# leonsick/depthg

Hardware: AMD Instinct MI355X
Metric: correlation-loss steps/sec at B=32,C=384,28x28 (fwd+bwd, per-GPU batch 32) (higher is better)
Workload: dtype bf16 (feats) / f16 (code) MFMA inputs, f32 accumulate

## Files before the change

depthg_amd/csrc/dg_api_corr.hip:

```cpp
#include "dg_api.h"
#include "dg_corr_args.h"
#include "dg_taps.h"

static unsigned long long* g_prof_span = nullptr;
extern "C" int dg_prof_main_span(void* span) { g_prof_span = static_cast<unsigned long long*>(span); return DG_OK; }

enum class Prep { Small, Dense, General };
enum class Sampler { Plane, ChannelLast };
enum class MainKernel { Small, Corr2, CorrMain };
enum class Depth { None, Job, GsBlocks, GsOwnLaunch };
enum class Hist { Rows, Blobs };
enum class Masks { None, Sampled, DenseRaw, DenseSplit };

struct PairSet {
    int op;
    int neg;
    bool mapped;
    float shift;
    int slot_loss, slot_cd;
    float fin_scale;
    int gidx, csel, dest;
    float factor;
};
struct Operand {
// ... 19 lines not shown
    float shift_depth;
    float inv_numel;
    float grad_f, grad_fn;
    int blob, blob_off_c;
    PairSet ps[DG_MAX_NEG + 2];
    Operand ops[DG_MAX_NEG + 2];
    bool gr_on;
    int gr_nkeys, gr_cpb, gr_blocks_per_image;
    int8_t gr_key[DG_MAX_JOBS], gr_first[DG_MAX_JOBS];
    int32_t gr_nblk[DG_MAX_JOBS];
    size_t nhwc_f[2], nhwc_c[2];
    size_t rows_f[DG_MAX_NEG + 2], rows_c[DG_MAX_NEG + 2];
    size_t op[DG_MAX_NEG + 2], inv[DG_MAX_NEG + 2], colpart[DG_MAX_NEG + 2], bbar[DG_MAX_NEG + 2];
    size_t ccolpart[DG_MAX_NEG + 2], csum[DG_MAX_NEG + 2], bsplit[DG_MAX_NEG + 2];
    size_t rvec[DG_MAX_NEG + 2], rimg[DG_MAX_NEG + 2];
    size_t nz, nzsum;
    size_t dRA[DG_MAX_NEG + 3], dRB[DG_MAX_NEG + 2];
    size_t part[DG_MAX_NEG + 3];
    size_t comb[2], scratch_out, taps, gbuf[DG_MAX_NEG + 2];
    size_t ticket;
    size_t maskbits[DG_MAX_NEG + 2];
    size_t clo[2];
    size_t gr_list, gr_count, gr_rank;
    size_t dRA2[DG_MAX_NEG + 2], dRBs[DG_MAX_NEG + 2], dRB2[DG_MAX_NEG + 2][2], dRBm[DG_MAX_NEG + 2], part4, om;
    size_t total;

    bool small() const { return prep == Prep::Small; }
    bool dense() const { return prep == Prep::Dense; }
    bool plane() const { return sampler == Sampler::Plane; }
    bool has_masks() const { return masks != Masks::None; }
    bool depth_in_gs() const { return depth_run == Depth::GsBlocks || depth_run == Depth::GsOwnLaunch; }
    bool dense_masks() const { return masks == Masks::DenseRaw || masks == Masks::DenseSplit; }
    bool intra_symmetric() const { return !pointwise || fold; }
    const int64_t* batch_map(int k, const int64_t* perms) const {
        return k < 0 ? nullptr : reinterpret_cast<const int64_t*>(reinterpret_cast<uintptr_t>(perms) + (size_t)k * B * sizeof(int64_t));
    }
    const int64_t* map_of(int t, const int64_t* perms) const { return batch_map(ps[t].mapped ? ps[t].neg : -1, perms); }
};

static inline float* f32(char* ws, size_t off) { return reinterpret_cast<float*>(ws + off); }

#define FOLD_STASH_OFF (5 * 1024)

static void plan_tables(const dg_corr_desc* d, Plan& p) {
    const double numel = (double)p.B * p.P * p.P;
    p.inv_numel = (float)(1.0 / numel);
// ... 109 lines not shown
    for (int i = 0; i < 2; ++i) p.comb[i] = take(B * p.Ppad * p.KD * 4);
    p.scratch_out = take(DG_OUT_COUNT * 4);
    p.taps = take(2 * B * dg_taps_record_bytes(p.hc * p.wc, p.P));
    for (int t = 0; t < p.T; ++t) p.gbuf[t] = p.grad ? take(B * (size_t)(p.Ppad / 32) * (p.Ppad / 32) * 2048) : 0;
    p.ticket = take(256);
    const bool xmask = rows && !p.small() && p.grad && plain_zero_clamp && p.Ppad <= 256 && p.rf == 4;
    const bool xmask_dense = (d->flags & DG_EXACT_MASKS) && ident && p.grad && plain_zero_clamp &&
                             p.KF == 384 && p.KD == 96 && p.D <= 80 && p.Ppad >= 160 && p.B <= 64;
    if ((d->flags & DG_EXACT_MASKS) && p.grad && (d->flags & DG_ZERO_CLAMP) && !xmask && !xmask_dense && !p.small())
        return fail(DG_ERR_UNSUPPORTED, "DG_EXACT_MASKS: exact clamp masks exist on small sample grids (always on there) and on the dense "
                                        "identity grid with C <= 384 (padded to 384), D <= 80, P >= 160, B <= 64, zero_clamp without stabalize");
    p.masks = xmask ? Masks::Sampled : (!xmask_dense ? Masks::None : (p.pointwise ? Masks::DenseSplit : Masks::DenseRaw));
    for (int t = 0; t < p.T; ++t) p.maskbits[t] = take(p.has_masks() ? B * (size_t)(p.Ppad / 32) * p.Ppad * 4 : 0);
    p.main = p.small() ? MainKernel::Small
                       : (p.grad && dg_corr2_shape_supported(p.KF, p.KD, p.D, p.lo, p.hi, p.Ppad, p.B) ? MainKernel::Corr2 : MainKernel::CorrMain);
    static const bool fold_on = [] { const char* e = getenv("DG_FOLD_INTRA"); return !(e && e[0] == '0'); }();
    p.fold = fold_on && p.main == MainKernel::Corr2 && p.pointwise && !xmask;
    p.half = p.main == MainKernel::Corr2 && ident && p.N * p.B <= 512 && p.S == p.h && p.S == p.w;
    p.depth_run = (!p.depth || p.small()) ? Depth::None : (!p.grad ? Depth::Job : (p.dense_masks() ? Depth::GsOwnLaunch : Depth::GsBlocks));
    for (int i = 0; i < 2; ++i) p.clo[i] = take(p.masks == Masks::DenseSplit ? B * (size_t)(p.Ppad / 32) * p.KD * 64 : 0);
    p.gr_list = take((size_t)DG_MAX_JOBS * B * DG_GR_CAP * 4);
    p.gr_count = take((size_t)DG_MAX_JOBS * B * 4);
    p.gr_rank = take((size_t)DG_MAX_JOBS * B * 2);
    {
        const bool sg = p.small() && p.grad, two = sg && p.pointwise;
        const size_t gt = B * p.Ppad * p.KD * 4;
        for (int t = 0; t < p.T; ++t) {
            p.dRA2[t] = take(two ? gt : 0);
            p.dRBs[t] = take(sg && p.nsplit == 2 ? gt : 0);
            for (int k = 0; k < 2; ++k) p.dRB2[t][k] = take(two && k < p.nsplit ? gt : 0);
            p.dRBm[t] = take(sg && t >= 2 && (p.pointwise || p.nsplit == 2) ? gt : 0);
        }
        p.part4 = take(p.small() ? (size_t)(p.T + 1) * B * p.nsplit * 16 : 0);
        p.om = take(p.small() ? (size_t)(p.T + 1) * 4 : 0);
    }
    p.total = off;
    plan_tables(d, p);
    return DG_OK;
}

extern "C" size_t dg_corr_workspace_bytes(const dg_corr_desc* desc) {
    Plan p{};
    if (make_plan(desc, p) != DG_OK) return 0;
    return p.total;
}

// ... 310 lines not shown
    DG_HIP(dg_launch_gather(g, p.KF, c.stream));
    return DG_OK;
}

static int fwd_colmeans(Fwd& c) {
    const Plan& p = c.p;
    const DgCorrArgs& a = c.a;
    DgColmeanArgs m;
    memset(&m, 0, sizeof(m));
    m.nops = p.nops; m.B = p.B; m.P = p.P; m.Ppad = p.Ppad; m.KF = p.KF; m.KD = p.KD;
    for (int o = 0; o < p.nops; ++o) {
        m.colpart[o] = p.pointwise ? f32(c.ws, p.colpart[o]) : nullptr; m.bbar[o] = f32(c.ws, p.bbar[o]);
        m.bsplit[o] = reinterpret_cast<__bf16*>(c.ws + p.bsplit[o]);
        m.ngroups[o] = p.Ppad / 32;
        m.ccolpart[o] = f32(c.ws, p.ccolpart[o]); m.csum[o] = f32(c.ws, p.csum[o]);
    }
    m.zero_word = p.depth_in_gs() ? reinterpret_cast<unsigned int*>(c.ws + p.ticket) : nullptr;
    m.zero_words9 = a.wctr;
    if (p.gr_on) {
        m.gr.nh = p.T; m.gr.nkeys = p.gr_nkeys; m.gr.B = p.B;
        for (int t = 0; t < p.T; ++t) { m.gr.sidx[t] = p.map_of(t, c.perms); m.gr.key[t] = p.gr_key[t]; }
        m.gr.list = reinterpret_cast<int32_t*>(c.ws + p.gr_list); m.gr.count = reinterpret_cast<int32_t*>(c.ws + p.gr_count);
        m.gr.rank = reinterpret_cast<int16_t*>(c.ws + p.gr_rank);
    }
    if (p.dense() && p.pointwise) {
        m.dc.code[0] = c.code; m.dc.code[1] = c.code_pos;
        for (int o = 0; o < 2; ++o) { m.dc.blob[o] = c.ws + p.op[o]; m.dc.inv_norm[o] = f32(c.ws, p.inv[o]); m.dc.ccolpart[o] = f32(c.ws, p.ccolpart[o]); }
        m.dc.B = p.B; m.dc.D = p.D; m.dc.KF = p.KF; m.dc.KD = p.KD; m.dc.h = p.h; m.dc.w = p.w; m.dc.P = p.P; m.dc.Ppad = p.Ppad;
        if (p.masks == Masks::DenseSplit) { m.dc.clo[0] = c.ws + p.clo[0]; m.dc.clo[1] = c.ws + p.clo[1]; }
    }
    if (c.split) {
        DgColmeanArgs ms = m;
        ms.zsel = 1; m.zsel = 2;
        DG_HIP(c.side->hand_over(0));
        DG_HIP(dg_launch_colmean(ms, c.side->stream()));
    }
    DG_HIP(dg_launch_colmean(m, c.stream));
    return DG_OK;
}

static int fwd_cd_mask3(Fwd& c) {
    const Plan& p = c.p;
    DgCdMask3Args m;
    memset(&m, 0, sizeof(m));
    m.opR = c.ws + p.op[0]; m.loR = c.ws + p.clo[0];
    for (int t = 0; t < p.T; ++t) {
// ... 220 lines not shown
    if (!p.grad) return fail(DG_ERR_INVALID, "dg_corr_backward needs a descriptor with DG_NEED_GRAD (as used in forward)");
    if (!coords1 || !coords2 || !grad_code || !grad_code_pos || !workspace) return fail(DG_ERR_INVALID, "null pointer");
    if (p.N > 0 && !perms) return fail(DG_ERR_INVALID, "perms is null with n_neg=%d", p.N);
    if (workspace_bytes < p.total) return fail(DG_ERR_WORKSPACE, "workspace %zu < required %zu bytes", workspace_bytes, p.total);
    char* ws = static_cast<char*>(workspace);
    DgScatterArgs s;
    memset(&s, 0, sizeof(s));
    ScatterFill fill{s, ws};
    if (p.small()) scatter_sources_small(p, perms, fill);
    else scatter_sources_blobs(p, perms, fill);
    if (p.depth) fill.add(p.dRA[p.T], nullptr, 3, 0, 2.0f * p.grad_f, 0, 1);
    s.coords1 = coords1; s.coords2 = coords2; s.gscal = grad_scalars; s.gtot = grad_total;
    s.wtot[0] = desc->w_intra; s.wtot[1] = desc->w_inter; s.wtot[2] = desc->w_neg; s.wtot[3] = desc->w_depth;
    s.comb[0] = f32(ws, p.comb[0]); s.comb[1] = f32(ws, p.comb[1]);
    s.taps = ws + p.taps;
    s.xop = ws + p.op[0]; s.xinv = f32(ws, p.inv[0]); s.blob_bytes = p.blob; s.blob_off_c = p.blob_off_c;
    s.xinv_dest[0] = f32(ws, p.inv[0]); s.xinv_dest[1] = p.nops > 1 ? f32(ws, p.inv[1]) : nullptr;
    s.out[0] = grad_code; s.out[1] = grad_code_pos;
    s.B = p.B; s.D = p.D; s.DP = p.KD; s.h = p.hc; s.w = p.wc; s.S = p.S; s.Sh = p.Sh; s.P = p.P; s.Ppad = p.Ppad;
    if ((size_t)p.hc * p.wc > 4096) return fail(DG_ERR_UNSUPPORTED, "code map %dx%d too large for the gradient gather (max 4096 pixels)", p.hc, p.wc);
    s.DC = 8;
    s.dense = p.dense() ? 1 : 0;
    s.taps_ready = p.dense() ? 0 : 1;
    DG_HIP(dg_launch_scatter(s, static_cast<hipStream_t>(stream_)));
    return DG_OK;
}

extern "C" int dg_corr_backward(const dg_corr_desc* desc, const float* grad_scalars, const float* coords1,
                                const float* coords2, const int64_t* perms, float* grad_code, float* grad_code_pos,
                                void* workspace, size_t workspace_bytes, dg_stream_t stream_) {
    if (!grad_scalars) return fail(DG_ERR_INVALID, "null pointer");
    return corr_backward_impl(desc, grad_scalars, nullptr, coords1, coords2, perms, grad_code, grad_code_pos, workspace,
                              workspace_bytes, stream_);
}

extern "C" int dg_corr_backward_total(const dg_corr_desc* desc, const float* grad_total, const float* coords1,
                                      const float* coords2, const int64_t* perms, float* grad_code, float* grad_code_pos,
                                      void* workspace, size_t workspace_bytes, dg_stream_t stream_) {
    if (!grad_total) return fail(DG_ERR_INVALID, "null pointer");
    return corr_backward_impl(desc, nullptr, grad_total, coords1, coords2, perms, grad_code, grad_code_pos, workspace,
                              workspace_bytes, stream_);
}

static int materialize_impl(const dg_corr_desc* desc, int32_t which, const int64_t* perms, float* out_cd, float* out_loss,
                            void* workspace, size_t workspace_bytes, dg_stream_t stream_) {
    Plan p{};
// ... 80 lines not shown
    int rc = make_plan(desc, p);
    if (rc != DG_OK) return rc;
    if (!workspace || workspace_bytes < p.total) return fail(DG_ERR_WORKSPACE, "workspace missing or too small");
    if (p.N > 0 && !perms) return fail(DG_ERR_INVALID, "perms is null");
    char* ws = static_cast<char*>(workspace);
    if (p.small()) {
        DgSmallArgs m;
        small_args(p, desc, ws, perms, m);
        m.out = f32(ws, p.scratch_out);
        DG_HIP(dg_launch_corr_small(m, static_cast<hipStream_t>(stream_)));
        return DG_OK;
    }
    DgCorrArgs a;
    build_corr_jobs(p, ws, perms, a);
    return launch_main(p, a, static_cast<hipStream_t>(stream_));
}

extern "C" int dg_corr_intra_folded(const dg_corr_desc* desc) {
    Plan p{};
    if (make_plan(desc, p) != DG_OK) return -1;
    return p.fold ? 1 : 0;
}

extern "C" const char* dg_corr_main_kernel_name(const dg_corr_desc* desc) {
    Plan p{};
    if (make_plan(desc, p) != DG_OK) return nullptr;
    return p.main == MainKernel::Small ? "k_corr_small" : (p.main == MainKernel::Corr2 ? "k_corr2" : "k_corr_main");
}

extern "C" int dg_normalize_split(int32_t B, int32_t C, int32_t h, int32_t w, const float* src, int32_t nchunks, int32_t chunk_c,
                                  float* const* dst, dg_stream_t stream_) {
    if (B < 1 || C < 1 || h < 1 || w < 1 || !src || !dst) return fail(DG_ERR_INVALID, "dg_normalize_split: bad arguments");
    if (nchunks < 1 || nchunks > 16 || chunk_c < 1 || (long long)chunk_c * (nchunks - 1) >= C || (long long)chunk_c * nchunks < C)
        return fail(DG_ERR_INVALID, "dg_normalize_split: %d chunks of %d channels do not tile C=%d (at most 16 chunks)", nchunks, chunk_c, C);
    for (int k = 0; k < nchunks; ++k) if (!dst[k]) return fail(DG_ERR_INVALID, "dg_normalize_split: null destination %d", k);
    DG_HIP(dg_launch_normalize_split(src, B, C, h * w, nchunks, chunk_c, dst, static_cast<hipStream_t>(stream_)));
    return DG_OK;
}
```

depthg_amd/csrc/dg_corr_args.h:

```cpp
#pragma once
#include "dg_device.h"

__host__ __device__ inline int dg_perm32(int pl) {
    int s = pl >> 4, u = (pl >> 3) & 1, hh = (pl >> 2) & 1, v = pl & 3;
    return (2 * s + hh) * 8 + 4 * u + v;
}

#ifndef DG_F_IG
#define DG_F_IG 4
#endif
__host__ __device__ inline int dg_f_off(int q, int g) {
    constexpr int IG = DG_F_IG;
    return ((g / IG) * 32 + q) * (IG * 16) + (((g % IG) ^ ((q / (16 / IG)) % IG)) * 16);
}

struct DgBlob {
    int GF, GD, KD;
    int off_c, off_p, bytes;
    __host__ __device__ DgBlob(int KF, int KD_) : GF(KF / 8), GD(KD_ / 8), KD(KD_) {
        off_c = 32 * GF * 16;
        off_p = off_c + GD * 32 * 16;
        bytes = off_p + 4 * KD * 16;
    }
    __host__ __device__ int f(int q, int g) const { return dg_f_off(q, g); }
// ... 315 lines not shown
    const int B = g.B;
    int src[DG_MAX_JOBS];
#pragma unroll
    for (int j = 0; j < DG_MAX_JOBS; ++j) {
        const bool mine = j < g.nh && g.key[j] == key && lane < B;
        const int64_t* sidx = mine ? g.sidx[j] : nullptr;
        src[j] = mine ? (sidx ? (int)sidx[lane] : lane) : -1;
    }
    int cnt = 0;
#pragma unroll
    for (int j = 0; j < DG_MAX_JOBS; ++j) {
        const bool hit = src[j] == m;
        const unsigned long long mask = __ballot(hit);
        if (hit) {
            const int rk = cnt + __popcll(mask & ((1ull << lane) - 1ull));
            g.rank[j * B + lane] = (int16_t)(rk < 32767 ? rk : 32767);
            if (rk < DG_GR_CAP) g.list[(key * B + m) * DG_GR_CAP + rk] = j | (lane << 8);
        }
        cnt += __popcll(mask);
    }
    if (lane == 0) g.count[key * B + m] = cnt < DG_GR_CAP ? cnt : DG_GR_CAP;
}

struct DgColmeanArgs {
    const float* colpart[DG_MAX_NEG + 2];
    float* bbar[DG_MAX_NEG + 2];
    __bf16* bsplit[DG_MAX_NEG + 2];
    const float* ccolpart[DG_MAX_NEG + 2];
    float* csum[DG_MAX_NEG + 2];
    int32_t ngroups[DG_MAX_NEG + 2];
    int32_t nops, B, P, Ppad, KF, KD;
    unsigned int* zero_word;
    unsigned int* zero_words9;
    DgGroupArgs gr;
    DgDenseCodeArgs dc;
    int32_t zsel;
};

struct DgRowmeanJob {
    const char* A;
    const float* bbar;
    const __bf16* bsplit;
    const int64_t* aidx;
    const int64_t* bidx;
    float* rvec;
    float* rimg;
};
struct DgRowmeanArgs {
    DgRowmeanJob jobs[DG_MAX_NEG + 2];
    int32_t njobs, B, P, Ppad, KF, KD;
    const float* abar;
    char* stash;
    int32_t stash_off;
    const float* cs_part[2];
    float* cs_out[2];
    int32_t ncs;
};
// ... 12 lines not shown
#define DG_MAX_SCATTER 48
struct DgScatterArgs {
    DgScatterSrc src[DG_MAX_SCATTER];
    int32_t nsrc;
    const float* coords1;
    const float* coords2;
    const float* gscal;
    const float* gtot;
    float wtot[4];
    float* comb[2];
    char* taps;
    const char* xop;
    const float* xinv;
    const float* xinv_dest[2];
    int32_t blob_bytes, blob_off_c;
    float* out[2];
    int32_t B, D, DP, h, w, S, Sh, P, Ppad, DC;
    int32_t dense;
    int8_t craw[2][DG_MAX_SCATTER / 2], cfin[2][DG_MAX_SCATTER / 2];
    int8_t ncraw[2], ncfin[2];
    int8_t crawh[2][DG_MAX_SCATTER / 2], cfinh[2][DG_MAX_SCATTER / 2];
    int8_t ncrawh[2], ncfinh[2];
    int32_t routed_half;
    int32_t taps_ready;
    int32_t naxpy;
    float* axo[DG_MAX_NEG + 2];
    const float* axd[DG_MAX_NEG + 2];
    const float* axd2[DG_MAX_NEG + 2];
    const float* axs[DG_MAX_NEG + 2];
    const float* axs2[DG_MAX_NEG + 2];
    const float* axf[DG_MAX_NEG + 2];
};

__device__ __forceinline__ float dg_src_factor(const DgScatterSrc& q) { return q.dfac ? q.factor * q.dfac[0] : q.factor; }
__device__ __forceinline__ float dg_gscal(const DgScatterArgs& a, int i) {
    return a.gscal ? a.gscal[i] + a.gscal[DG_OUT_TOTAL] * a.wtot[i] : a.gtot[0] * a.wtot[i];
}

struct DgGsJob {
    const uint16_t* G;
    const char* Rop;
    const char* Sop;
    const float* ScInv;
    const int64_t* ridx;
    const int64_t* sidx;
    float* dS;
// ... 66 lines not shown
```

depthg_amd/csrc/dg_post.hip:

```cpp
#include "dg_device.h"
#include "dg_corr_args.h"
#include "dg_taps.h"
#include <cstdlib>

typedef const float __attribute__((address_space(1)))* gfloat_p;


#define DG_LOAD_GS(a, gs)                                                                                   \
    float gs[4];                                                                                            \
    {                                                                                                       \
        const bool vec_ = (a).gscal != nullptr;                                                             \
        const float gt_ = vec_ ? (a).gscal[DG_OUT_TOTAL] : (a).gtot[0];                                     \
        const float g0_ = vec_ ? (a).gscal[0] : 0.f, g1_ = vec_ ? (a).gscal[1] : 0.f;                       \
        const float g2_ = vec_ ? (a).gscal[2] : 0.f, g3_ = vec_ ? (a).gscal[3] : 0.f;                       \
        gs[0] = g0_ + gt_ * (a).wtot[0]; gs[1] = g1_ + gt_ * (a).wtot[1];                                  \
        gs[2] = g2_ + gt_ * (a).wtot[2]; gs[3] = g3_ + gt_ * (a).wtot[3];                                  \
    }
__device__ __forceinline__ float dg_pick(const float (&gs)[4], int i) { return i == 0 ? gs[0] : (i == 1 ? gs[1] : (i == 2 ? gs[2] : gs[3])); }

template <int NDF>
__global__ __launch_bounds__(64 * NDF) void k_grad_combine(const DgScatterArgs a) {
    const int rt = blockIdx.x, n = blockIdx.y, dest = blockIdx.z;
    const int lane = threadIdx.x & 63, r = lane & 31, h = lane >> 5, DP = NDF * 32;
    const int d = __builtin_amdgcn_readfirstlane((int)threadIdx.x >> 6);
// ... 73 lines not shown
            v[i] = (v[i] - (float)x[0][i] * t) * inv;
        }
    }
    add_sources(a.cfin[dest], a.ncfin[dest]);
    if (ok) {
        float* out = a.comb[dest] + tile_off;
#pragma unroll
        for (int g = 0; g < 4; ++g) {
            const f32x4 t = {v[4 * g], v[4 * g + 1], v[4 * g + 2], v[4 * g + 3]};
            *reinterpret_cast<f32x4*>(out + g * 256) = t;
        }
    }
}

#ifndef COMB_HB_HM
#define COMB_HB_HM 4
#endif
#ifndef COMB_HB
#define COMB_HB 4
#endif
#define COMB_MAXROUTE 512
template <int NDF, bool HM = false>
__global__ __launch_bounds__(64 * NDF) void k_combine_out(const DgScatterArgs a) {
    const int rt = blockIdx.x, n = blockIdx.y, dest = blockIdx.z;
    const int tid = threadIdx.x, lane = tid & 63, r = lane & 31, h = lane >> 5, DP = NDF * 32;
    const int d = __builtin_amdgcn_readfirstlane(tid >> 6);
    __shared__ __attribute__((aligned(16))) char xs[NDF][DG_XROWS_LDS];
    __shared__ float part[NDF][32];
    __shared__ float stage[NDF][32 * 33];
    __shared__ const float* rl_p[COMB_MAXROUTE];
    __shared__ float rl_w[COMB_MAXROUTE];
    __shared__ int rl_cnt, wcnt[NDF], rsrc[DG_MAX_SCATTER];
    DG_LOAD_GS(a, gs)
    int nr = 0;
    for (int s = 0; s < a.nsrc; ++s)
        if (a.src[s].dest == dest && a.src[s].route != nullptr) { if (tid == 0) rsrc[nr] = s; ++nr; }
    if (tid == 0) rl_cnt = 0;
    __syncthreads();
    for (int i0 = 0; i0 < nr * a.B; i0 += 64 * NDF) {
        const int i = i0 + tid;
        bool hit = false;
        int m = 0, s = 0;
        if (i < nr * a.B) {
            const int rs = i / a.B;
            m = i - rs * a.B; s = rsrc[rs];
            hit = (int)a.src[s].route[m] == n;
        }
        const unsigned long long bal = __ballot(hit);
        if (lane == 0) wcnt[d] = __popcll(bal);
        __syncthreads();
        int base = rl_cnt;
        for (int wv = 0; wv < d; ++wv) base += wcnt[wv];
        if (hit) {
            const int o = base + __popcll(bal & ((1ull << lane) - 1));
            const DgScatterSrc& q = a.src[s];
            if (o < COMB_MAXROUTE) {
                rl_p[o] = q.half ? reinterpret_cast<const float*>(reinterpret_cast<const _Float16*>(q.buf) + (size_t)m * a.Ppad * a.DP) : q.buf + (size_t)m * a.Ppad * a.DP;
                rl_w[o] = dg_src_factor(q) * dg_pick(gs, q.gidx);
            }
        }
        __syncthreads();
        if (tid == 0) {
            int c = rl_cnt;
            for (int wv = 0; wv < NDF; ++wv) c += wcnt[wv];
            rl_cnt = min(c, COMB_MAXROUTE);
        }
        __syncthreads();
    }
    const int cnt = rl_cnt;
    const bool ok = 32 * d + r < a.D;
    const size_t in_img = (size_t)rt * (32 * DP) + lane * 4 + (ok ? d * 1024 : 0);
    const size_t tile_off = (size_t)n * a.Ppad * DP + in_img;
    float v[16];
#pragma unroll
    for (int i = 0; i < 16; ++i) v[i] = 0.f;
    const size_t in_img_h = (size_t)rt * (32 * DP) + lane * 8 + (ok ? d * 1024 : 0);
    constexpr int HB = HM ? COMB_HB_HM : COMB_HB, FB = HM ? 1 : 4;
    float invd[16];
#pragma unroll
    for (int i = 0; i < 16; ++i) {
        const int rr = rt * 32 + (i & 3) + 8 * (i >> 2) + 4 * h;
        invd[i] = (a.xinv_dest[dest] && rr < a.P) ? a.xinv_dest[dest][(size_t)n * a.Ppad + rr] : 0.f;
    }
    const _Float16 __attribute__((address_space(1)))* const hdummy = reinterpret_cast<const _Float16 __attribute__((address_space(1)))*>(reinterpret_cast<uintptr_t>(a.xinv));
    auto add_half4 = [&](const _Float16 __attribute__((address_space(1)))* const (&hb)[HB], const float (&sc)[HB], const bool raw) __attribute__((always_inline)) {
        f16x8 t0[HB], t1[HB];
#pragma unroll
        for (int u = 0; u < HB; ++u) {
            t0[u] = *reinterpret_cast<const f16x8 __attribute__((address_space(1)))*>(hb[u]);
            t1[u] = *reinterpret_cast<const f16x8 __attribute__((address_space(1)))*>(hb[u] + ((ok && hb[u] != hdummy) ? 512 : 0));
        }
#pragma unroll
        for (int u = 0; u < HB; ++u) {
            const bool use = ok && sc[u] != 0.f;
#pragma unroll
            for (int e = 0; e < 8; ++e) {
                v[e] = fmaf(raw ? sc[u] : sc[u] * invd[e], use ? (float)t0[u][e] : 0.f, v[e]);
                v[8 + e] = fmaf(raw ? sc[u] : sc[u] * invd[8 + e], use ? (float)t1[u][e] : 0.f, v[8 + e]);
            }
        }
    };
    auto add_sources_half = [&](const int8_t* list, const int nsrc_, const bool raw) __attribute__((always_inline)) {
        for (int k0 = 0; k0 < nsrc_; k0 += HB) {
            const _Float16 __attribute__((address_space(1)))* hb[HB];
            float sc[HB];
#pragma unroll
            for (int u = 0; u < HB; ++u) {
                const bool live = k0 + u < nsrc_;
                const DgScatterSrc& q = a.src[(int)list[live ? k0 + u : k0]];
                sc[u] = live ? dg_src_factor(q) * dg_pick(gs, q.gidx) : 0.f;
                hb[u] = live ? reinterpret_cast<const _Float16 __attribute__((address_space(1)))*>(reinterpret_cast<uintptr_t>(q.buf)) + (size_t)n * a.Ppad * DP + in_img_h
                             : hdummy;
            }
            add_half4(hb, sc, raw);
        }
    };
    auto add_sources = [&](const int8_t* list, const int nsrc_) __attribute__((always_inline)) {

        for (int k0 = 0; k0 < nsrc_; k0 += FB) {
            f32x4 t[FB][4];
            float sc[FB];
#pragma unroll
            for (int u = 0; u < FB; ++u) {
                const bool live = k0 + u < nsrc_;
                const DgScatterSrc& q = a.src[(int)list[live ? k0 + u : k0]];
                sc[u] = live ? dg_src_factor(q) * dg_pick(gs, q.gidx) : 0.f;
                const float* base = q.buf + tile_off;
#pragma unroll
                for (int g = 0; g < 4; ++g) t[u][g] = *reinterpret_cast<const f32x4*>(base + (ok ? g * 256 : 0));
            }
#pragma unroll
            for (int u = 0; u < FB; ++u) {
                const bool use = ok && k0 + u < nsrc_;
#pragma unroll
                for (int g = 0; g < 4; ++g)
#pragma unroll
                    for (int e = 0; e < 4; ++e) v[4 * g + e] = fmaf(sc[u], use ? t[u][g][e] : 0.f, v[4 * g + e]);
            }
        }
    };
    const int nraw = a.ncraw[dest] + a.ncrawh[dest];
    add_sources(a.craw[dest], a.ncraw[dest]);
    add_sources_half(a.crawh[dest], a.ncrawh[dest], true);
    if (nraw > 0) {
        const char* xb = a.xop + ((size_t)n * (a.Ppad >> 5) + rt) * a.blob_bytes + a.blob_off_c + d * 2048;
        _Float16 x[1][16];
        dg_load_code_rows<1>(xb, xs[d], lane, x);
#pragma unroll
        for (int i = 0; i < 16; ++i) {
            const float t = half_sum((float)x[0][i] * v[i]);
            if (r == 0) part[d][h * 16 + i] = t;
        }
        __syncthreads();
#pragma unroll
        for (int i = 0; i < 16; ++i) {
            float t = part[0][h * 16 + i];
#pragma unroll
            for (int f = 1; f < NDF; ++f) t += part[f][h * 16 + i];
            const int rr = rt * 32 + (i & 3) + 8 * (i >> 2) + 4 * h;
            const float inv = rr < a.P ? a.xinv[(size_t)n * a.Ppad + rr] : 0.f;
            v[i] = (v[i] - (float)x[0][i] * t) * inv;
        }
    }
    add_sources(a.cfin[dest], a.ncfin[dest]);
    add_sources_half(a.cfinh[dest], a.ncfinh[dest], false);
    if (a.routed_half) {
        for (int e0 = 0; e0 < cnt; e0 += HB) {
            const _Float16 __attribute__((address_space(1)))* hb[HB];
            float sc[HB];
#pragma unroll
            for (int k = 0; k < HB; ++k) {
                const int e = min(e0 + k, cnt - 1);
                sc[k] = e0 + k < cnt ? rl_w[e] : 0.f;
                hb[k] = sc[k] != 0.f ? reinterpret_cast<const _Float16 __attribute__((address_space(1)))*>(reinterpret_cast<uintptr_t>(rl_p[e])) + in_img_h : hdummy;
            }
            add_half4(hb, sc, false);
        }
    } else
    for (int e0 = 0; e0 < cnt; e0 += 4) {
        f32x4 u4[4][4];
        float sc[4];
#pragma unroll
        for (int k = 0; k < 4; ++k) {
            const int e = min(e0 + k, cnt - 1);
            sc[k] = e0 + k < cnt ? rl_w[e] : 0.f;
            const gfloat_p sb = (gfloat_p)rl_p[e] + in_img;
#pragma unroll
            for (int g = 0; g < 4; ++g) u4[k][g] = *(const f32x4 __attribute__((address_space(1)))*)(sb + (ok ? g * 256 : 0));
        }
#pragma unroll
        for (int k = 0; k < 4; ++k)
#pragma unroll
            for (int g = 0; g < 4; ++g)
#pragma unroll
                for (int e = 0; e < 4; ++e) v[4 * g + e] = fmaf(sc[k], ok ? u4[k][g][e] : 0.f, v[4 * g + e]);
    }
    float* st = stage[d];
#pragma unroll
    for (int i = 0; i < 16; ++i) st[r * 33 + (i & 3) + 8 * (i >> 2) + 4 * h] = v[i];
    __builtin_amdgcn_fence(__ATOMIC_RELEASE, "workgroup");
    __builtin_amdgcn_wave_barrier();
    __builtin_amdgcn_fence(__ATOMIC_ACQUIRE, "workgroup");
    const int HW = a.h * a.w, p = rt * 32 + r;
    float* out = a.out[dest] + (size_t)n * a.D * HW + p;
#pragma unroll
    for (int it = 0; it < 16; ++it) {
        const int c = 2 * it + h, ch = 32 * d + c;
        if (ch < a.D && p < a.P) out[(size_t)ch * HW] = st[c * 33 + r];
    }
// ... 364 lines not shown

hipError_t dg_launch_scatter(const DgScatterArgs& a, hipStream_t s) {
    DgScatterArgs ac = a;
    {
        for (int dest = 0; dest < 2; ++dest) {
            ac.ncraw[dest] = ac.ncfin[dest] = ac.ncrawh[dest] = ac.ncfinh[dest] = 0;
            for (int i = 0; i < a.nsrc; ++i) {
                const DgScatterSrc& q = a.src[i];
                if (q.dest != dest || q.route != nullptr) continue;
                int8_t& cnt = q.half ? (q.raw ? ac.ncrawh[dest] : ac.ncfinh[dest]) : (q.raw ? ac.ncraw[dest] : ac.ncfin[dest]);
                if (cnt >= DG_MAX_SCATTER / 2) return hipErrorInvalidValue;
                (q.half ? (q.raw ? ac.crawh[dest] : ac.cfinh[dest]) : (q.raw ? ac.craw[dest] : ac.cfin[dest]))[cnt++] = (int8_t)i;
            }
        }
        const dim3 cgrid(a.Ppad / 32, a.B, 2);
        {
            int nrouted = 0;
            for (int i = 0; i < a.nsrc; ++i) nrouted += a.src[i].route != nullptr;
            bool any_half = false;
            int routed_h = 0;
            for (int i = 0; i < a.nsrc; ++i) { any_half = any_half || a.src[i].half != 0; routed_h += (a.src[i].route != nullptr && a.src[i].half) ? 1 : 0; }
            if (routed_h != 0 && routed_h != nrouted) return hipErrorInvalidValue;
            ac.routed_half = routed_h != 0 ? 1 : 0;
            const bool one_launch = a.dense && a.S == a.h && a.S == a.w && nrouted * a.B <= COMB_MAXROUTE && (a.DP == 96 || a.DP == 128);
            if (any_half && !one_launch) return hipErrorInvalidValue;
            if (one_launch) {
                if (a.DP == 96 && any_half) hipLaunchKernelGGL((k_combine_out<3, true>), cgrid, dim3(192), 0, s, ac);
                else if (a.DP == 96) hipLaunchKernelGGL(k_combine_out<3>, cgrid, dim3(192), 0, s, ac);
                else hipLaunchKernelGGL(k_combine_out<4>, cgrid, dim3(256), 0, s, ac);
                return hipGetLastError();
            }
        }
        const dim3 cgrid2(a.Ppad / 32, a.B, 2 + a.naxpy);
        if (a.DP == 96) hipLaunchKernelGGL(k_grad_combine<3>, cgrid2, dim3(192), 0, s, ac);
        else if (a.DP == 128) hipLaunchKernelGGL(k_grad_combine<4>, cgrid2, dim3(256), 0, s, ac);
        else return hipErrorInvalidValue;
    }
    const int HW = a.h * a.w;
    {
        int nrouted = 0;
        for (int i = 0; i < a.nsrc; ++i) nrouted += a.src[i].route != nullptr;
        int CGv = 16;
        auto stage_bytes = [&](int cg) { return (size_t)cg * (HW + 2) * 4 + (size_t)DENSE_MAXROUTE * 12; };
        if (stage_bytes(CGv) > 150 * 1024 && CGv > 8) CGv = 8;
        const size_t dsm = stage_bytes(CGv);
        if (a.dense && a.S == a.h && a.S == a.w && dsm <= 150 * 1024 && (size_t)nrouted * a.B <= DENSE_MAXROUTE) {
            auto launch = [&](auto kern, int threads) -> hipError_t {
                hipError_t e = dg_set_max_smem(reinterpret_cast<const void*>(kern), (int)dsm);
                if (e != hipSuccess) return e;
                hipLaunchKernelGGL(kern, dim3(a.DP / CGv, a.B, 2), dim3(threads), dsm, s, a);
// ... 338 lines not shown
```

depthg_amd/csrc/dg_prep.hip:

```cpp
#include "dg_device.h"
#include "dg_corr_args.h"
#include "dg_taps.h"
#include <cstdlib>

__global__ void k_nchw_to_nhwc(const DgTransposeArgs a) {
    __shared__ float t[32][33];
    const int b = blockIdx.z;
    int m = 0, gy = blockIdx.y;
    while (m < a.nmaps - 1 && gy >= (a.K4[m] + 31) / 32) { gy -= (a.K4[m] + 31) / 32; ++m; }
    const float* __restrict__ src = a.src[m];
    float* __restrict__ dst = a.dst[m];
    const int K = a.K[m], K4 = a.K4[m], HW = a.HW[m];
    const int k0 = gy * 32, p0 = blockIdx.x * 32;
    if (p0 >= HW) return;
    const int tx = threadIdx.x, ty = threadIdx.y;
    for (int i = ty; i < 32; i += 8) {
        int k = k0 + i, p = p0 + tx;
        t[i][tx] = (k < K && p < HW) ? src[((size_t)b * K + k) * HW + p] : 0.f;
    }
    __syncthreads();
    for (int i = ty; i < 32; i += 8) {
        int p = p0 + i, k = k0 + tx;
        if (p < HW && k < K4) dst[((size_t)b * HW + p) * K4 + k] = t[tx][i];
    }
// ... 911 lines not shown
            for (int u = 0; u < 4; ++u) v[u] = cp[(size_t)(t + u) * K];
#pragma unroll
            for (int u = 0; u < 4; ++u) s += v[u];
        }
        for (; t < ngroups; ++t) s += cp[(size_t)t * K];
        out[(size_t)n * K + k] = s * scale;
    }
}

__global__ __launch_bounds__(256) void k_colmean(const DgColmeanArgs a) {
    extern __shared__ __attribute__((aligned(16))) char cm_smem[];
    const int n = blockIdx.x, o = blockIdx.y;
    if (a.zero_word && n == 0 && o == 0 && blockIdx.z == 0 && threadIdx.x == 0) *a.zero_word = 0u;
    if (a.zero_words9 && n == 0 && o == 0 && blockIdx.z == 0 && threadIdx.x < 9) a.zero_words9[threadIdx.x] = 0u;
    auto reduce = [&](const float* part, int ngroups, int K, float scale, float* out) __attribute__((always_inline)) { colsum_reduce(part, n, ngroups, K, scale, out); };
    if (a.zsel == 1 ? blockIdx.z != 3 : (a.zsel == 2 && blockIdx.z == 3)) return;
    if (blockIdx.z == 3) {
        const int GD = a.dc.KD / 8;
        if ((int)blockIdx.y < 2 * GD) dense_code_planes(a.dc, cm_smem, n, (int)blockIdx.y / GD, (int)blockIdx.y % GD);
        return;
    }
    if (blockIdx.z == 2) {
        if ((int)blockIdx.y < a.gr.nkeys && threadIdx.x < 64) dg_group_lists(a.gr, n, o, threadIdx.x);
        return;
    }
    if (o >= a.nops) return;
    if (blockIdx.z == 0 && a.colpart[o]) {
        reduce(a.colpart[o], a.ngroups[o], a.KF, 1.f / (float)a.P, a.bbar[o]);
        __syncthreads();
        for (int k = threadIdx.x; k < a.KF; k += 256) {
            const float v = a.bbar[o][(size_t)n * a.KF + k];
            const __bf16 hi = (__bf16)v;
            a.bsplit[o][((size_t)n * 2) * a.KF + k] = hi;
            a.bsplit[o][((size_t)n * 2 + 1) * a.KF + k] = (__bf16)(v - (float)hi);
        }
    }
    if (blockIdx.z == 1 && a.ccolpart[o] && a.dc.B == 0) reduce(a.ccolpart[o], a.Ppad / 32, a.KD, 1.f, a.csum[o]);
}

hipError_t dg_launch_colmean(const DgColmeanArgs& a, hipStream_t s) {
    int ny = a.gr.nkeys > a.nops ? a.gr.nkeys : a.nops;
    int nz = a.gr.nkeys > 0 ? 3 : 2, smem = 0;
    if (a.dc.B > 0) {
        if (a.nops != 2) return hipErrorInvalidValue;
        ny = max(ny, 2 * (a.dc.KD / 8)); nz = 4; smem = a.dc.Ppad * 16 * ((a.dc.clo[0] || a.dc.clo[1]) ? 2 : 1);
        hipError_t e = dg_set_max_smem(reinterpret_cast<const void*>(k_colmean), smem);
        if (e != hipSuccess) return e;
    }
    hipLaunchKernelGGL(k_colmean, dim3(a.B, ny, nz), dim3(256), smem, s, a);
    return hipGetLastError();
}

#define ROWMEAN_WAVES 4
__global__ __launch_bounds__(64 * ROWMEAN_WAVES) void k_rowmean(const DgRowmeanArgs a) {
    extern __shared__ __attribute__((aligned(16))) char rm_smem[];
    const int tile = blockIdx.x, n = blockIdx.y, tid = threadIdx.x, lane = tid & 63, c = lane & 31, h = lane >> 5;
    const int wid = __builtin_amdgcn_readfirstlane(tid >> 6);
    const int KF = a.KF, nt = a.Ppad / 32;
    if (tile == nt + 1) {
        for (int o = 0; o < a.ncs; ++o) colsum_reduce(a.cs_part[o], n, nt, a.KD, 1.f, a.cs_out[o]);
        return;
    }
    if (tile == nt) {
        float av[12];
#pragma unroll
// ... 94 lines not shown
```

Measured before the change: 3354.

## Precompute routed-source lists in colmean and prefetch half sources in combine

Builds per-(dest,image) routing lists ahead of time in an extra wave of the colmean kernel, so k_combine_out reads a precomputed count and list instead of scanning route maps with ballots and several block barriers. The half-precision combine path is also restructured to issue loads for the first raw and first final/routed batches early, overlapping them with the code-row projection. This adds workspace for the lists and extra validation, and makes combine depend on colmean having written the lists.

```diff
diff --git a/depthg_amd/csrc/dg_api_corr.hip b/depthg_amd/csrc/dg_api_corr.hip
--- a/depthg_amd/csrc/dg_api_corr.hip
+++ b/depthg_amd/csrc/dg_api_corr.hip
@@ -65,6 +65,8 @@
     size_t maskbits[DG_MAX_NEG + 2];
     size_t clo[2];
     size_t gr_list, gr_count, gr_rank;
+    bool rl_on;
+    size_t rl_list, rl_count;
     size_t dRA2[DG_MAX_NEG + 2], dRBs[DG_MAX_NEG + 2], dRB2[DG_MAX_NEG + 2][2], dRBm[DG_MAX_NEG + 2], part4, om;
     size_t total;
 
@@ -220,6 +222,9 @@
     p.gr_list = take((size_t)DG_MAX_JOBS * B * DG_GR_CAP * 4);
     p.gr_count = take((size_t)DG_MAX_JOBS * B * 4);
     p.gr_rank = take((size_t)DG_MAX_JOBS * B * 2);
+    p.rl_on = p.half && p.N > 0 && p.B % 8 == 0 && p.B <= 64;
+    p.rl_count = take(p.rl_on ? 2 * B * 4 : 0);
+    p.rl_list = take(p.rl_on ? 2 * B * p.N * B * 4 : 0);
     {
         const bool sg = p.small() && p.grad, two = sg && p.pointwise;
         const size_t gt = B * p.Ppad * p.KD * 4;
@@ -576,6 +581,11 @@
         for (int t = 0; t < p.T; ++t) { m.gr.sidx[t] = p.map_of(t, c.perms); m.gr.key[t] = p.gr_key[t]; }
         m.gr.list = reinterpret_cast<int32_t*>(c.ws + p.gr_list); m.gr.count = reinterpret_cast<int32_t*>(c.ws + p.gr_count);
         m.gr.rank = reinterpret_cast<int16_t*>(c.ws + p.gr_rank);
+    }
+    if (p.rl_on) {
+        m.rl.nr[0] = p.N; m.rl.B = p.B; m.rl.stride = p.N * p.B;
+        for (int k = 0; k < p.N; ++k) m.rl.map[0][k] = p.batch_map(k, c.perms);
+        m.rl.list = reinterpret_cast<int32_t*>(c.ws + p.rl_list); m.rl.count = reinterpret_cast<int32_t*>(c.ws + p.rl_count);
     }
     if (p.dense() && p.pointwise) {
         m.dc.code[0] = c.code; m.dc.code[1] = c.code_pos;
@@ -842,6 +852,10 @@
     s.DC = 8;
     s.dense = p.dense() ? 1 : 0;
     s.taps_ready = p.dense() ? 0 : 1;
+    if (p.rl_on) {
+        s.rl_list = reinterpret_cast<const int32_t*>(ws + p.rl_list); s.rl_count = reinterpret_cast<const int32_t*>(ws + p.rl_count);
+        s.rl_stride = p.N * p.B; s.rl_nr[0] = (int8_t)p.N;
+    }
     DG_HIP(dg_launch_scatter(s, static_cast<hipStream_t>(stream_)));
     return DG_OK;
 }
@@ -968,6 +982,12 @@
     return p.fold ? 1 : 0;
 }
 
+extern "C" long long dg_corr_route_list_bytes(const dg_corr_desc* desc) {
+    Plan p{};
+    if (make_plan(desc, p) != DG_OK) return -1;
+    return p.rl_on ? (long long)(up((size_t)2 * p.B * 4, 256) + up((size_t)2 * p.B * p.N * p.B * 4, 256)) : 0;
+}
+
 extern "C" const char* dg_corr_main_kernel_name(const dg_corr_desc* desc) {
     Plan p{};
     if (make_plan(desc, p) != DG_OK) return nullptr;
diff --git a/depthg_amd/csrc/dg_corr_args.h b/depthg_amd/csrc/dg_corr_args.h
--- a/depthg_amd/csrc/dg_corr_args.h
+++ b/depthg_amd/csrc/dg_corr_args.h
@@ -361,6 +361,34 @@
     if (lane == 0) g.count[key * B + m] = cnt < DG_GR_CAP ? cnt : DG_GR_CAP;
 }
 
+struct DgRouteListArgs {
+    const int64_t* map[2][DG_MAX_NEG];
+    int32_t nr[2];
+    int32_t B, stride;
+    int32_t* list;
+    int32_t* count;
+};
+__device__ __forceinline__ void dg_route_list(const DgRouteListArgs& g, const int n, const int dest, const int lane) {
+    const int B = g.B, nr = g.nr[dest];
+    int to[DG_MAX_NEG];
+#pragma unroll
+    for (int k = 0; k < DG_MAX_NEG; ++k) {
+        const bool mine = k < nr && lane < B;
+        const int64_t* map = mine ? g.map[dest][k] : nullptr;
+        to[k] = mine ? (int)map[lane] : -1;
+    }
+    int32_t* out = g.list + ((size_t)dest * B + n) * g.stride;
+    int cnt = 0;
+#pragma unroll
+    for (int k = 0; k < DG_MAX_NEG; ++k) {
+        const bool hit = to[k] == n;
+        const unsigned long long mask = __ballot(hit);
+        if (hit) out[cnt + __popcll(mask & ((1ull << lane) - 1ull))] = k | (lane << 8);
+        cnt += __popcll(mask);
+    }
+    if (lane == 0) g.count[dest * B + n] = cnt;
+}
+
 struct DgColmeanArgs {
     const float* colpart[DG_MAX_NEG + 2];
     float* bbar[DG_MAX_NEG + 2];
@@ -372,6 +400,7 @@
     unsigned int* zero_word;
     unsigned int* zero_words9;
     DgGroupArgs gr;
+    DgRouteListArgs rl;
     DgDenseCodeArgs dc;
     int32_t zsel;
 };
@@ -430,6 +459,11 @@
     int8_t crawh[2][DG_MAX_SCATTER / 2], cfinh[2][DG_MAX_SCATTER / 2];
     int8_t ncrawh[2], ncfinh[2];
     int32_t routed_half;
+    const int32_t* rl_list;
+    const int32_t* rl_count;
+    int32_t rl_stride;
+    int8_t rl_nr[2], nrouted[2];
+    int8_t rl_src[2][DG_MAX_NEG];
     int32_t taps_ready;
     int32_t naxpy;
     float* axo[DG_MAX_NEG + 2];
diff --git a/depthg_amd/csrc/dg_post.hip b/depthg_amd/csrc/dg_post.hip
--- a/depthg_amd/csrc/dg_post.hip
+++ b/depthg_amd/csrc/dg_post.hip
@@ -119,6 +119,8 @@
 #define COMB_MAXROUTE 512
 template <int NDF, bool HM = false>
 __global__ __launch_bounds__(64 * NDF) void k_combine_out(const DgScatterArgs a) {
+    typedef const _Float16 __attribute__((address_space(1)))* ghalf_p;
+    typedef const int32_t __attribute__((address_space(4)))* cint_p;
     const int rt = blockIdx.x, n = blockIdx.y, dest = blockIdx.z;
     const int tid = threadIdx.x, lane = tid & 63, r = lane & 31, h = lane >> 5, DP = NDF * 32;
     const int d = __builtin_amdgcn_readfirstlane(tid >> 6);
@@ -129,42 +131,62 @@
     __shared__ float rl_w[COMB_MAXROUTE];
     __shared__ int rl_cnt, wcnt[NDF], rsrc[DG_MAX_SCATTER];
     DG_LOAD_GS(a, gs)
-    int nr = 0;
-    for (int s = 0; s < a.nsrc; ++s)
-        if (a.src[s].dest == dest && a.src[s].route != nullptr) { if (tid == 0) rsrc[nr] = s; ++nr; }
-    if (tid == 0) rl_cnt = 0;
-    __syncthreads();
-    for (int i0 = 0; i0 < nr * a.B; i0 += 64 * NDF) {
-        const int i = i0 + tid;
-        bool hit = false;
-        int m = 0, s = 0;
-        if (i < nr * a.B) {
-            const int rs = i / a.B;
-            m = i - rs * a.B; s = rsrc[rs];
-            hit = (int)a.src[s].route[m] == n;
-        }
-        const unsigned long long bal = __ballot(hit);
-        if (lane == 0) wcnt[d] = __popcll(bal);
-        __syncthreads();
-        int base = rl_cnt;
-        for (int wv = 0; wv < d; ++wv) base += wcnt[wv];
-        if (hit) {
-            const int o = base + __popcll(bal & ((1ull << lane) - 1));
-            const DgScatterSrc& q = a.src[s];
-            if (o < COMB_MAXROUTE) {
-                rl_p[o] = q.half ? reinterpret_cast<const float*>(reinterpret_cast<const _Float16*>(q.buf) + (size_t)m * a.Ppad * a.DP) : q.buf + (size_t)m * a.Ppad * a.DP;
-                rl_w[o] = dg_src_factor(q) * dg_pick(gs, q.gidx);
-            }
-        }
-        __syncthreads();
-        if (tid == 0) {
-            int c = rl_cnt;
-            for (int wv = 0; wv < NDF; ++wv) c += wcnt[wv];
-            rl_cnt = min(c, COMB_MAXROUTE);
-        }
-        __syncthreads();
-    }
-    const int cnt = rl_cnt;
+    const bool fed = a.rl_list != nullptr;
+    const cint_p rl = reinterpret_cast<cint_p>(reinterpret_cast<uintptr_t>(a.rl_list + ((size_t)dest * a.B + n) * a.rl_stride));
+    int cnt = 0;
+    if (a.nrouted[dest] > 0) {
+        if (fed) {
+            cnt = max(0, min((int)reinterpret_cast<cint_p>(reinterpret_cast<uintptr_t>(a.rl_count))[dest * a.B + n], min(a.rl_stride, COMB_MAXROUTE)));
+        } else {
+            int nr = 0;
+            for (int s = 0; s < a.nsrc; ++s)
+                if (a.src[s].dest == dest && a.src[s].route != nullptr) { if (tid == 0) rsrc[nr] = s; ++nr; }
+            if (tid == 0) rl_cnt = 0;
+            __syncthreads();
+            for (int i0 = 0; i0 < nr * a.B; i0 += 64 * NDF) {
+                const int i = i0 + tid;
+                bool hit = false;
+                int m = 0, s = 0;
+                if (i < nr * a.B) {
+                    const int rs = i / a.B;
+                    m = i - rs * a.B; s = rsrc[rs];
+                    hit = (int)a.src[s].route[m] == n;
+                }
+                const unsigned long long bal = __ballot(hit);
+                if (lane == 0) wcnt[d] = __popcll(bal);
+                __syncthreads();
+                int base = rl_cnt;
+                for (int wv = 0; wv < d; ++wv) base += wcnt[wv];
+                if (hit) {
+                    const int o = base + __popcll(bal & ((1ull << lane) - 1));
+                    const DgScatterSrc& q = a.src[s];
+                    if (o < COMB_MAXROUTE) {
+                        rl_p[o] = q.half ? reinterpret_cast<const float*>(reinterpret_cast<const _Float16*>(q.buf) + (size_t)m * a.Ppad * a.DP) : q.buf + (size_t)m * a.Ppad * a.DP;
+                        rl_w[o] = dg_src_factor(q) * dg_pick(gs, q.gidx);
+                    }
+                }
+                __syncthreads();
+                if (tid == 0) {
+                    int c = rl_cnt;
+                    for (int wv = 0; wv < NDF; ++wv) c += wcnt[wv];
+                    rl_cnt = min(c, COMB_MAXROUTE);
+                }
+                __syncthreads();
+            }
+            cnt = rl_cnt;
+        }
+    }
+    auto rl_get = [&](const int e, const float*& p, float& w) __attribute__((always_inline)) {
+        if (fed) {
+            const unsigned ent = (unsigned)rl[e];
+            const DgScatterSrc& q = a.src[(int)a.rl_src[dest][min(ent & 255u, (unsigned)a.nrouted[dest] - 1u)]];
+            const size_t off = (size_t)min(ent >> 8, (unsigned)a.B - 1u) * a.Ppad * a.DP;
+            p = q.half ? reinterpret_cast<const float*>(reinterpret_cast<const _Float16*>(q.buf) + off) : q.buf + off;
+            w = dg_src_factor(q) * dg_pick(gs, q.gidx);
+        } else {
+            p = rl_p[e]; w = rl_w[e];
+        }
+    };
     const bool ok = 32 * d + r < a.D;
     const size_t in_img = (size_t)rt * (32 * DP) + lane * 4 + (ok ? d * 1024 : 0);
     const size_t tile_off = (size_t)n * a.Ppad * DP + in_img;
@@ -179,14 +201,15 @@
         const int rr = rt * 32 + (i & 3) + 8 * (i >> 2) + 4 * h;
         invd[i] = (a.xinv_dest[dest] && rr < a.P) ? a.xinv_dest[dest][(size_t)n * a.Ppad + rr] : 0.f;
     }
-    const _Float16 __attribute__((address_space(1)))* const hdummy = reinterpret_cast<const _Float16 __attribute__((address_space(1)))*>(reinterpret_cast<uintptr_t>(a.xinv));
-    auto add_half4 = [&](const _Float16 __attribute__((address_space(1)))* const (&hb)[HB], const float (&sc)[HB], const bool raw) __attribute__((always_inline)) {
-        f16x8 t0[HB], t1[HB];
+    const ghalf_p hdummy = reinterpret_cast<ghalf_p>(reinterpret_cast<uintptr_t>(a.xinv));
+    auto load_half = [&](const ghalf_p (&hb)[HB], f16x8 (&t0)[HB], f16x8 (&t1)[HB]) __attribute__((always_inline)) {
 #pragma unroll
         for (int u = 0; u < HB; ++u) {
             t0[u] = *reinterpret_cast<const f16x8 __attribute__((address_space(1)))*>(hb[u]);
             t1[u] = *reinterpret_cast<const f16x8 __attribute__((address_space(1)))*>(hb[u] + ((ok && hb[u] != hdummy) ? 512 : 0));
         }
+    };
+    auto use_half = [&](const f16x8 (&t0)[HB], const f16x8 (&t1)[HB], const float (&sc)[HB], const bool raw) __attribute__((always_inline)) {
 #pragma unroll
         for (int u = 0; u < HB; ++u) {
             const bool use = ok && sc[u] != 0.f;
@@ -197,24 +220,40 @@
             }
         }
     };
-    auto add_sources_half = [&](const int8_t* list, const int nsrc_, const bool raw) __attribute__((always_inline)) {
-        for (int k0 = 0; k0 < nsrc_; k0 += HB) {
-            const _Float16 __attribute__((address_space(1)))* hb[HB];
+    auto add_half4 = [&](const ghalf_p (&hb)[HB], const float (&sc)[HB], const bool raw) __attribute__((always_inline)) {
+        f16x8 t0[HB], t1[HB];
+        load_half(hb, t0, t1);
+        use_half(t0, t1, sc, raw);
+    };
+    auto half_batch = [&](const int8_t* list, const int nsrc_, const int k0, ghalf_p (&hb)[HB], float (&sc)[HB]) __attribute__((always_inline)) {
+#pragma unroll
+        for (int u = 0; u < HB; ++u) {
+            const bool live = k0 + u < nsrc_;
+            const DgScatterSrc& q = a.src[(int)list[live ? k0 + u : 0]];
+            sc[u] = live ? dg_src_factor(q) * dg_pick(gs, q.gidx) : 0.f;
+            hb[u] = live ? reinterpret_cast<ghalf_p>(reinterpret_cast<uintptr_t>(q.buf)) + (size_t)n * a.Ppad * DP + in_img_h : hdummy;
+        }
+    };
+    auto add_sources_half = [&](const int8_t* list, const int nsrc_, const bool raw, const int kfirst) __attribute__((always_inline)) {
+        for (int k0 = kfirst; k0 < nsrc_; k0 += HB) {
+            ghalf_p hb[HB];
             float sc[HB];
-#pragma unroll
-            for (int u = 0; u < HB; ++u) {
-                const bool live = k0 + u < nsrc_;
-                const DgScatterSrc& q = a.src[(int)list[live ? k0 + u : k0]];
-                sc[u] = live ? dg_src_factor(q) * dg_pick(gs, q.gidx) : 0.f;
-                hb[u] = live ? reinterpret_cast<const _Float16 __attribute__((address_space(1)))*>(reinterpret_cast<uintptr_t>(q.buf)) + (size_t)n * a.Ppad * DP + in_img_h
-                             : hdummy;
-            }
+            half_batch(list, nsrc_, k0, hb, sc);
             add_half4(hb, sc, raw);
         }
     };
-    auto add_sources = [&](const int8_t* list, const int nsrc_) __attribute__((always_inline)) {
-
-        for (int k0 = 0; k0 < nsrc_; k0 += FB) {
+    auto routed_batch = [&](const int e0, const int cnt_, ghalf_p (&hb)[HB], float (&sc)[HB]) __attribute__((always_inline)) {
+#pragma unroll
+        for (int k = 0; k < HB; ++k) {
+            const float* p = nullptr;
+            float w = 0.f;
+            if (e0 + k < cnt_) rl_get(e0 + k, p, w);
+            sc[k] = w;
+            hb[k] = w != 0.f ? reinterpret_cast<ghalf_p>(reinterpret_cast<uintptr_t>(p)) + in_img_h : hdummy;
+        }
+    };
+    auto add_sources = [&](const int8_t* list, const int nsrc_, const int kfirst) __attribute__((always_inline)) {
+        for (int k0 = kfirst; k0 < nsrc_; k0 += FB) {
             f32x4 t[FB][4];
             float sc[FB];
 #pragma unroll
@@ -236,52 +275,135 @@
             }
         }
     };
-    const int nraw = a.ncraw[dest] + a.ncrawh[dest];
-    add_sources(a.craw[dest], a.ncraw[dest]);
-    add_sources_half(a.crawh[dest], a.ncrawh[dest], true);
-    if (nraw > 0) {
-        const char* xb = a.xop + ((size_t)n * (a.Ppad >> 5) + rt) * a.blob_bytes + a.blob_off_c + d * 2048;
-        _Float16 x[1][16];
-        dg_load_code_rows<1>(xb, xs[d], lane, x);
+    const int nrawf = a.ncraw[dest], nrawh = a.ncrawh[dest], nraw = nrawf + nrawh;
+    const char* xb = a.xop + ((size_t)n * (a.Ppad >> 5) + rt) * a.blob_bytes + a.blob_off_c + d * 2048;
+    auto project_sums = [&](const _Float16 (&x)[16]) __attribute__((always_inline)) {
 #pragma unroll
         for (int i = 0; i < 16; ++i) {
-            const float t = half_sum((float)x[0][i] * v[i]);
+            const float t = half_sum((float)x[i] * v[i]);
             if (r == 0) part[d][h * 16 + i] = t;
         }
+    };
+    auto project = [&](const _Float16 (&x)[16], const float (&inv)[16]) __attribute__((always_inline)) {
         __syncthreads();
 #pragma unroll
         for (int i = 0; i < 16; ++i) {
             float t = part[0][h * 16 + i];
 #pragma unroll
             for (int f = 1; f < NDF; ++f) t += part[f][h * 16 + i];
-            const int rr = rt * 32 + (i & 3) + 8 * (i >> 2) + 4 * h;
-            const float inv = rr < a.P ? a.xinv[(size_t)n * a.Ppad + rr] : 0.f;
-            v[i] = (v[i] - (float)x[0][i] * t) * inv;
-        }
-    }
-    add_sources(a.cfin[dest], a.ncfin[dest]);
-    add_sources_half(a.cfinh[dest], a.ncfinh[dest], false);
-    if (a.routed_half) {
-        for (int e0 = 0; e0 < cnt; e0 += HB) {
-            const _Float16 __attribute__((address_space(1)))* hb[HB];
-            float sc[HB];
-#pragma unroll
-            for (int k = 0; k < HB; ++k) {
-                const int e = min(e0 + k, cnt - 1);
-                sc[k] = e0 + k < cnt ? rl_w[e] : 0.f;
-                hb[k] = sc[k] != 0.f ? reinterpret_cast<const _Float16 __attribute__((address_space(1)))*>(reinterpret_cast<uintptr_t>(rl_p[e])) + in_img_h : hdummy;
-            }
-            add_half4(hb, sc, false);
-        }
-    } else
+            v[i] = (v[i] - (float)x[i] * t) * inv[i];
+        }
+    };
+    if constexpr (HM) {
+        const char* const xdummy = reinterpret_cast<const char*>(a.xinv);
+        i32x4 xraw[2];
+#pragma unroll
+        for (int k = 0; k < 2; ++k) xraw[k] = *reinterpret_cast<const i32x4*>(nraw > 0 ? xb + k * 1024 + lane * 16 : xdummy);
+        f32x4 tf[4];
+        float scf;
+        {
+            const bool live = nrawf > 0;
+            const DgScatterSrc& q = a.src[(int)a.craw[dest][0]];
+            scf = live ? dg_src_factor(q) * dg_pick(gs, q.gidx) : 0.f;
+            const float* base = live ? q.buf + tile_off : a.xinv;
+#pragma unroll
+            for (int g = 0; g < 4; ++g) tf[g] = *reinterpret_cast<const f32x4*>(base + ((ok && live) ? g * 256 : 0));
+        }
+        ghalf_p hb0[HB];
+        float sc0[HB];
+        f16x8 t0[HB], t1[HB];
+        {
+            const bool use = ok && nrawf > 0;
+#pragma unroll
+            for (int g = 0; g < 4; ++g)
+#pragma unroll
+                for (int e = 0; e < 4; ++e) v[4 * g + e] = fmaf(scf, use ? tf[g][e] : 0.f, v[4 * g + e]);
+        }
+        add_sources(a.craw[dest], nrawf, FB);
+        half_batch(a.crawh[dest], nrawh, 0, hb0, sc0);
+        load_half(hb0, t0, t1);
+        use_half(t0, t1, sc0, true);
+        add_sources_half(a.crawh[dest], nrawh, true, HB);
+        const int nfinh = a.ncfinh[dest];
+        const bool pre_routed = nfinh == 0 && a.routed_half;
+        auto request_next = [&]() __attribute__((always_inline)) {
+            if (pre_routed) routed_batch(0, cnt, hb0, sc0);
+            else half_batch(a.cfinh[dest], nfinh, 0, hb0, sc0);
+            load_half(hb0, t0, t1);
+        };
+        if (nraw > 0) {
+            _Float16 x[16];
+            char* T = xs[d];
+#pragma unroll
+            for (int k = 0; k < 2; ++k) {
+                const int L = k * 64 + lane;
+                *reinterpret_cast<i32x4*>(T + ((L >> 5) * 33 + (L & 31)) * 16) = xraw[k];
+            }
+#pragma unroll
+            for (int i = 0; i < 16; ++i) {
+                const int q = (i & 3) + 8 * (i >> 2) + 4 * h;
+                x[i] = *reinterpret_cast<const _Float16*>(T + ((r >> 3) * 33 + q) * 16 + (r & 7) * 2);
+            }
+            project_sums(x);
+            if (a.xinv_dest[dest] == a.xinv) project(x, invd);
+            else {
+                float inv[16];
+#pragma unroll
+                for (int i = 0; i < 16; ++i) {
+                    const int rr = rt * 32 + (i & 3) + 8 * (i >> 2) + 4 * h;
+                    inv[i] = rr < a.P ? a.xinv[(size_t)n * a.Ppad + rr] : 0.f;
+                }
+                project(x, inv);
+            }
+        }
+        request_next();
+        add_sources(a.cfin[dest], a.ncfin[dest], 0);
+        use_half(t0, t1, sc0, false);
+        add_sources_half(a.cfinh[dest], nfinh, false, HB);
+        if (a.routed_half) {
+            for (int e0 = pre_routed ? HB : 0; e0 < cnt; e0 += HB) {
+                routed_batch(e0, cnt, hb0, sc0);
+                add_half4(hb0, sc0, false);
+            }
+        }
+    } else {
+        add_sources(a.craw[dest], nrawf, 0);
+        add_sources_half(a.crawh[dest], nrawh, true, 0);
+        if (nraw > 0) {
+            _Float16 x[1][16];
+            dg_load_code_rows<1>(xb, xs[d], lane, x);
+            float inv[16];
+#pragma unroll
+            for (int i = 0; i < 16; ++i) {
+                const int rr = rt * 32 + (i & 3) + 8 * (i >> 2) + 4 * h;
+                inv[i] = rr < a.P ? a.xinv[(size_t)n * a.Ppad + rr] : 0.f;
+            }
+            project_sums(x[0]);
+            project(x[0], inv);
+        }
+        add_sources(a.cfin[dest], a.ncfin[dest], 0);
+        add_sources_half(a.cfinh[dest], a.ncfinh[dest], false, 0);
+        if (a.routed_half) {
+            for (int e0 = 0; e0 < cnt; e0 += HB) {
+                ghalf_p hb[HB];
+                float sc[HB];
+                routed_batch(e0, cnt, hb, sc);
+                add_half4(hb, sc, false);
+            }
+        }
+    }
+    if constexpr (!HM)
+    if (!a.routed_half)
     for (int e0 = 0; e0 < cnt; e0 += 4) {
         f32x4 u4[4][4];
         float sc[4];
 #pragma unroll
         for (int k = 0; k < 4; ++k) {
-            const int e = min(e0 + k, cnt - 1);
-            sc[k] = e0 + k < cnt ? rl_w[e] : 0.f;
-            const gfloat_p sb = (gfloat_p)rl_p[e] + in_img;
+            const float* p = nullptr;
+            float w = 0.f;
+            rl_get(min(e0 + k, cnt - 1), p, w);
+            sc[k] = e0 + k < cnt ? w : 0.f;
+            const gfloat_p sb = (gfloat_p)p + in_img;
 #pragma unroll
             for (int g = 0; g < 4; ++g) u4[k][g] = *(const f32x4 __attribute__((address_space(1)))*)(sb + (ok ? g * 256 : 0));
         }
@@ -692,10 +814,20 @@
             for (int i = 0; i < a.nsrc; ++i) { any_half = any_half || a.src[i].half != 0; routed_h += (a.src[i].route != nullptr && a.src[i].half) ? 1 : 0; }
             if (routed_h != 0 && routed_h != nrouted) return hipErrorInvalidValue;
             ac.routed_half = routed_h != 0 ? 1 : 0;
+            int nrd[2] = {0, 0};
+            for (int i = 0; i < a.nsrc; ++i) {
+                const DgScatterSrc& q = a.src[i];
+                if (q.route == nullptr || q.dest < 0 || q.dest > 1) continue;
+                if (nrd[q.dest] < DG_MAX_NEG) ac.rl_src[q.dest][nrd[q.dest]] = (int8_t)i;
+                ++nrd[q.dest];
+            }
+            ac.nrouted[0] = (int8_t)nrd[0]; ac.nrouted[1] = (int8_t)nrd[1];
+            if (a.rl_list && (!a.rl_count || nrd[0] > DG_MAX_NEG || nrd[1] > DG_MAX_NEG || nrd[0] != a.rl_nr[0] || nrd[1] != a.rl_nr[1] || a.rl_stride < a.B * (nrd[0] > nrd[1] ? nrd[0] : nrd[1])))
+                return hipErrorInvalidValue;
             const bool one_launch = a.dense && a.S == a.h && a.S == a.w && nrouted * a.B <= COMB_MAXROUTE && (a.DP == 96 || a.DP == 128);
             if (any_half && !one_launch) return hipErrorInvalidValue;
             if (one_launch) {
-                if (a.DP == 96 && any_half) hipLaunchKernelGGL((k_combine_out<3, true>), cgrid, dim3(192), 0, s, ac);
+                if (a.DP == 96 && any_half && (nrouted == 0 || routed_h != 0)) hipLaunchKernelGGL((k_combine_out<3, true>), cgrid, dim3(192), 0, s, ac);
                 else if (a.DP == 96) hipLaunchKernelGGL(k_combine_out<3>, cgrid, dim3(192), 0, s, ac);
                 else hipLaunchKernelGGL(k_combine_out<4>, cgrid, dim3(256), 0, s, ac);
                 return hipGetLastError();
diff --git a/depthg_amd/csrc/dg_prep.hip b/depthg_amd/csrc/dg_prep.hip
--- a/depthg_amd/csrc/dg_prep.hip
+++ b/depthg_amd/csrc/dg_prep.hip
@@ -957,6 +957,7 @@
     }
     if (blockIdx.z == 2) {
         if ((int)blockIdx.y < a.gr.nkeys && threadIdx.x < 64) dg_group_lists(a.gr, n, o, threadIdx.x);
+        if (o < 2 && (threadIdx.x >> 6) == 1 && a.rl.nr[o] > 0) dg_route_list(a.rl, n, o, threadIdx.x & 63);
         return;
     }
     if (o >= a.nops) return;
@@ -975,7 +976,11 @@
 
 hipError_t dg_launch_colmean(const DgColmeanArgs& a, hipStream_t s) {
     int ny = a.gr.nkeys > a.nops ? a.gr.nkeys : a.nops;
-    int nz = a.gr.nkeys > 0 ? 3 : 2, smem = 0;
+    const bool lists = a.rl.nr[0] > 0 || a.rl.nr[1] > 0;
+    if (lists && (a.rl.B != a.B || a.B > 64 || a.rl.nr[0] > DG_MAX_NEG || a.rl.nr[1] > DG_MAX_NEG ||
+                  a.rl.stride < a.B * max(a.rl.nr[0], a.rl.nr[1]))) return hipErrorInvalidValue;
+    if (lists && ny < 2) ny = 2;
+    int nz = (a.gr.nkeys > 0 || lists) ? 3 : 2, smem = 0;
     if (a.dc.B > 0) {
         if (a.nops != 2) return hipErrorInvalidValue;
         ny = max(ny, 2 * (a.dc.KD / 8)); nz = 4; smem = a.dc.Ppad * 16 * ((a.dc.clo[0] || a.dc.clo[1]) ? 2 : 1);
```

Result: no change. 3360, median of 2 (+0.2%).
